# raymondclowe/EasyWakeWord

Measured on AMD Instinct MI355X. Metric: real-time 16 kHz streams sustained + MFCC frames/sec at 1/2/4/8 GPUs, higher is better.
Workload: dtype fp32

## Files before the change

### easywakeword_amd/csrc/ewk_mfcc_dft.h

```cpp
#pragma once
#include <hip/hip_runtime.h>

namespace ewk {

#define EWK_LD128(r, a, c) asm volatile("ds_read_b128 %0, %1 offset:%2" : "=v"(r[c]) : "v"(a), "i"(16 * (c)) : "memory")
#define EWK_LD128_8(r, addr)                                                                        \
    do {                                                                                           \
        const uint32_t _a = (addr);                                                                \
        EWK_LD128(r, _a, 0); EWK_LD128(r, _a, 1); EWK_LD128(r, _a, 2); EWK_LD128(r, _a, 3);         \
        EWK_LD128(r, _a, 4); EWK_LD128(r, _a, 5); EWK_LD128(r, _a, 6); EWK_LD128(r, _a, 7);         \
    } while (0)
#define EWK_WAIT_8(r)                                                                              \
    asm volatile("s_waitcnt lgkmcnt(0)" : "+v"(r[0]), "+v"(r[1]), "+v"(r[2]), "+v"(r[3]), "+v"(r[4]), \
                 "+v"(r[5]), "+v"(r[6]), "+v"(r[7]) : : "memory")

__device__ __forceinline__ float2 cmul(float2 a, float2 w) {
    return make_float2(a.x * w.x - a.y * w.y, a.x * w.y + a.y * w.x);
}

__device__ __forceinline__ void dft4(float2& a0, float2& a1, float2& a2, float2& a3) {
    const float2 t0 = make_float2(a0.x + a2.x, a0.y + a2.y);
    const float2 t1 = make_float2(a0.x - a2.x, a0.y - a2.y);
    const float2 t2 = make_float2(a1.x + a3.x, a1.y + a3.y);
    const float2 t3 = make_float2(a1.x - a3.x, a1.y - a3.y);
    a0 = make_float2(t0.x + t2.x, t0.y + t2.y);
    a2 = make_float2(t0.x - t2.x, t0.y - t2.y);
    a1 = make_float2(t1.x + t3.y, t1.y - t3.x);
    a3 = make_float2(t1.x - t3.y, t1.y + t3.x);
}

__device__ __forceinline__ void dft16_stage2(float2 (&x)[16]) {
    constexpr float C1 = 0.92387953251128674f, R2 = 0.70710678118654752f, T = 0.41421356237309505f;
    dft4(x[0], x[1], x[2], x[3]);
    {
        const float2 a0 = x[4], y1 = x[5], y2 = x[6], y3 = x[7];
        const float2 u2 = make_float2(y2.x + y2.y, y2.y - y2.x);
        const float2 t0 = make_float2(fmaf(R2, u2.x, a0.x), fmaf(R2, u2.y, a0.y));
        const float2 t1 = make_float2(fmaf(-R2, u2.x, a0.x), fmaf(-R2, u2.y, a0.y));
        const float2 u1 = make_float2(fmaf(T, y1.y, y1.x), fmaf(-T, y1.x, y1.y));
        const float2 u3 = make_float2(fmaf(T, y3.x, y3.y), fmaf(T, y3.y, -y3.x));
        const float2 v2 = make_float2(u1.x + u3.x, u1.y + u3.y), v3 = make_float2(u1.x - u3.x, u1.y - u3.y);
        x[4] = make_float2(fmaf(C1, v2.x, t0.x), fmaf(C1, v2.y, t0.y));
        x[6] = make_float2(fmaf(-C1, v2.x, t0.x), fmaf(-C1, v2.y, t0.y));
        x[5] = make_float2(fmaf(C1, v3.y, t1.x), fmaf(-C1, v3.x, t1.y));
        x[7] = make_float2(fmaf(-C1, v3.y, t1.x), fmaf(C1, v3.x, t1.y));
    }
    {
        const float2 a0 = x[8], y1 = x[9], y2 = x[10], y3 = x[11];
        const float2 t0 = make_float2(a0.x + y2.y, a0.y - y2.x);
        const float2 t1 = make_float2(a0.x - y2.y, a0.y + y2.x);
        const float2 u1 = make_float2(y1.x + y1.y, y1.y - y1.x);
        const float d3 = y3.y - y3.x, n3 = y3.x + y3.y;
        const float2 v2 = make_float2(u1.x + d3, u1.y - n3), v3 = make_float2(u1.x - d3, u1.y + n3);
        x[8] = make_float2(fmaf(R2, v2.x, t0.x), fmaf(R2, v2.y, t0.y));
        x[10] = make_float2(fmaf(-R2, v2.x, t0.x), fmaf(-R2, v2.y, t0.y));
        x[9] = make_float2(fmaf(R2, v3.y, t1.x), fmaf(-R2, v3.x, t1.y));
        x[11] = make_float2(fmaf(-R2, v3.y, t1.x), fmaf(R2, v3.x, t1.y));
    }
    {
        const float2 a0 = x[12], y1 = x[13], y2 = x[14], y3 = x[15];
        const float d2 = y2.y - y2.x, n2 = y2.x + y2.y;
        const float2 t0 = make_float2(fmaf(R2, d2, a0.x), fmaf(-R2, n2, a0.y));
        const float2 t1 = make_float2(fmaf(-R2, d2, a0.x), fmaf(R2, n2, a0.y));
        const float2 u1 = make_float2(fmaf(T, y1.x, y1.y), fmaf(T, y1.y, -y1.x));
        const float m3 = fmaf(T, y3.y, y3.x), u3y = fmaf(T, y3.x, -y3.y);
        const float2 v2 = make_float2(u1.x - m3, u1.y + u3y), v3 = make_float2(u1.x + m3, u1.y - u3y);
        x[12] = make_float2(fmaf(C1, v2.x, t0.x), fmaf(C1, v2.y, t0.y));
        x[14] = make_float2(fmaf(-C1, v2.x, t0.x), fmaf(-C1, v2.y, t0.y));
        x[13] = make_float2(fmaf(C1, v3.y, t1.x), fmaf(-C1, v3.x, t1.y));
        x[15] = make_float2(fmaf(-C1, v3.y, t1.x), fmaf(C1, v3.x, t1.y));
    }
}

__device__ __forceinline__ void dft16_perm(float2 (&x)[16]) {
#pragma unroll
    for (int n2 = 0; n2 < 4; ++n2) dft4(x[n2], x[4 + n2], x[8 + n2], x[12 + n2]);
    dft16_stage2(x);
}

__device__ __forceinline__ void dft16_perm_win(float2 (&x)[16], const float2 (&w)[16]) {
#pragma unroll
    for (int n2 = 0; n2 < 4; ++n2) {
        const float2 x0 = x[n2], x1 = x[4 + n2], x2 = x[8 + n2], x3 = x[12 + n2];
        const float2 w0 = w[n2], w1 = w[4 + n2], w2 = w[8 + n2], w3 = w[12 + n2];
        const float2 p2 = make_float2(x2.x * w2.x, x2.y * w2.y), p3 = make_float2(x3.x * w3.x, x3.y * w3.y);
        const float2 t0 = make_float2(fmaf(x0.x, w0.x, p2.x), fmaf(x0.y, w0.y, p2.y));
        const float2 t1 = make_float2(fmaf(x0.x, w0.x, -p2.x), fmaf(x0.y, w0.y, -p2.y));
        const float2 t2 = make_float2(fmaf(x1.x, w1.x, p3.x), fmaf(x1.y, w1.y, p3.y));
        const float2 t3 = make_float2(fmaf(x1.x, w1.x, -p3.x), fmaf(x1.y, w1.y, -p3.y));
        x[n2] = make_float2(t0.x + t2.x, t0.y + t2.y);
        x[8 + n2] = make_float2(t0.x - t2.x, t0.y - t2.y);
        x[4 + n2] = make_float2(t1.x + t3.y, t1.y - t3.x);
        x[12 + n2] = make_float2(t1.x - t3.y, t1.y + t3.x);
    }
    dft16_stage2(x);
}

__device__ __forceinline__ constexpr int dperm(int k) { return 4 * (k & 3) + (k >> 2); }

}
```

### easywakeword_amd/csrc/ewk_mfcc_fft.h

```cpp
#pragma once
#include <hip/hip_runtime.h>
#include <math.h>

#include "ewk_internal.h"
#include "ewk_mfcc_layout.h"
#include "ewk_mfcc_dft.h"
#include "ewk_mfcc_tile.h"

#define EWK_SETPRIO(v) __builtin_amdgcn_s_setprio(v)

namespace ewk {

__host__ __device__ constexpr int tr_off(int r, int h) {
    const int jp = r < 8 ? r : (r == 8 ? 0 : 16 - r);
    const int q = (jp >> 2) + (r >= 8 ? 2 : 0);
    return 64 * (16 * h + 4 * (jp & 3) + q) + 4 * ((jp & 3) + 8 * h);
}

template <int RING>
struct SegSrc {
    __amdgpu_buffer_rsrc_t rsrc;
    int32_t len;
    int32_t wrap_at;
    int32_t start;
    int32_t ring;
};

constexpr int sample_bytes(int ring) { return ring == 2 ? 2 : 4; }

template <int RING>
__device__ __forceinline__ SegSrc<RING> make_src(const void* p, int64_t start, int64_t ring, int32_t len) {
    SegSrc<RING> v;
    const unsigned char* b = static_cast<const unsigned char*>(p) + (RING ? 0 : start * sample_bytes(RING));
    const uint64_t bu = (uint64_t)b;
    const uint32_t lo = __builtin_amdgcn_readfirstlane((uint32_t)bu);
    const uint32_t hi = __builtin_amdgcn_readfirstlane((uint32_t)(bu >> 32));
    const void* bb = (const void*)(((uint64_t)hi << 32) | lo);
    const int32_t n = __builtin_amdgcn_readfirstlane(RING ? (int32_t)ring : len);
    v.rsrc = __builtin_amdgcn_make_buffer_rsrc((void*)bb, (short)0, n * sample_bytes(RING), 0x00020000);
    v.len = __builtin_amdgcn_readfirstlane(len);
    v.start = __builtin_amdgcn_readfirstlane((int32_t)start);
    v.ring = __builtin_amdgcn_readfirstlane((int32_t)ring);
    v.wrap_at = v.ring - v.start;
    return v;
}

template <int RING>
__device__ __forceinline__ void stage_load(const SegSrc<RING>& v, int q0, int lane, float (&r)[kStageLoads]) {
#pragma unroll
    for (int c = 0; c < kStageLoads; ++c) {
        const int q = q0 + 64 * c + lane;
        int off;
        if (RING) {
            const int phys = q >= v.wrap_at ? q - v.wrap_at : q + v.start;
            off = (unsigned)q < (unsigned)v.len ? phys * sample_bytes(RING) : -1;
        } else {
            off = q * 4;
        }
        if (RING == 2)
            r[c] = (float)(short)__builtin_amdgcn_raw_buffer_load_b16(v.rsrc, off, 0, 0);
        else
            r[c] = __builtin_bit_cast(float, __builtin_amdgcn_raw_buffer_load_b32(v.rsrc, off, 0, 0));
    }
}

#define EWK_ST13(o)                                                                                            \
    asm volatile("s_mov_b32 %[sv], m0\n\ts_mov_b32 m0, %[base]\n\ts_nop 0\n\t"                              \
                 "ds_write_addtid_b32 %[r0] offset:%[o0]\n\tds_write_addtid_b32 %[r1] offset:%[o1]\n\t"          \
                 "ds_write_addtid_b32 %[r2] offset:%[o2]\n\tds_write_addtid_b32 %[r3] offset:%[o3]\n\t"          \
                 "ds_write_addtid_b32 %[r4] offset:%[o4]\n\tds_write_addtid_b32 %[r5] offset:%[o5]\n\t"          \
                 "ds_write_addtid_b32 %[r6] offset:%[o6]\n\tds_write_addtid_b32 %[r7] offset:%[o7]\n\t"          \
                 "ds_write_addtid_b32 %[r8] offset:%[o8]\n\tds_write_addtid_b32 %[r9] offset:%[o9]\n\t"          \
                 "ds_write_addtid_b32 %[r10] offset:%[o10]\n\tds_write_addtid_b32 %[r11] offset:%[o11]\n\t"      \
                 "ds_write_addtid_b32 %[r12] offset:%[o12]\n\ts_mov_b32 m0, %[sv]"                                 \
                 : [sv] "=&s"(m0save)                                                                          \
                 : [base] "s"(m0base), [r0] "v"(r[o]), [r1] "v"(r[o + 1]), [r2] "v"(r[o + 2]), [r3] "v"(r[o + 3]), \
                   [r4] "v"(r[o + 4]), [r5] "v"(r[o + 5]), [r6] "v"(r[o + 6]), [r7] "v"(r[o + 7]),                \
                   [r8] "v"(r[o + 8]), [r9] "v"(r[o + 9]), [r10] "v"(r[o + 10]), [r11] "v"(r[o + 11]),          \
                   [r12] "v"(r[o + 12]), [o0] "i"(stg_off(o)), [o1] "i"(stg_off(o + 1)), [o2] "i"(stg_off(o + 2)), \
                   [o3] "i"(stg_off(o + 3)), [o4] "i"(stg_off(o + 4)), [o5] "i"(stg_off(o + 5)),                    \
                   [o6] "i"(stg_off(o + 6)), [o7] "i"(stg_off(o + 7)), [o8] "i"(stg_off(o + 8)),                    \
                   [o9] "i"(stg_off(o + 9)), [o10] "i"(stg_off(o + 10)), [o11] "i"(stg_off(o + 11)),                \
                   [o12] "i"(stg_off(o + 12))                                                                     \
                 : "memory")
static_assert(kStageLoads == 26, "stage_store writes two blocks of 13 rows");
__device__ __forceinline__ void stage_store(float* stage, int lane, const float (&r)[kStageLoads]) {
    const uint32_t m0base = __builtin_amdgcn_readfirstlane((uint32_t)(uintptr_t)stage);
    uint32_t m0save;
    EWK_ST13(0);
    EWK_ST13(13);
}

constexpr int kMelW[8] = {2, 2, 2, 3, 4, 6, 9, 12};
constexpr int kMelIt0[8] = {0, 2, 4, 6, 9, 13, 19, 28};
constexpr int kMelOff[8] = {0, 2, 4, 8, 12, 16, 24, 36};
constexpr int kMelRow = 48;
static_assert(kMelRow <= WP && WP % 4 == 0, "mel weight rows");

template <int G>
__device__ __forceinline__ void xpose_write(const float2 (&ag)[16], int half, uint32_t m0base) {
    constexpr int g = G;
    float w[16];
#pragma unroll
    for (int k1 = 0; k1 < 16; ++k1) w[k1] = half ? ag[dperm(k1)].y : ag[dperm(k1)].x;
    uint32_t m0save;
    asm volatile("s_mov_b32 %[sv], m0\n\ts_mov_b32 m0, %[base]\n\ts_nop 0\n\t"
                 "ds_write_addtid_b32 %[w0] offset:%[o0]\n\tds_write_addtid_b32 %[w1] offset:%[o1]\n\t"
                 "ds_write_addtid_b32 %[w2] offset:%[o2]\n\tds_write_addtid_b32 %[w3] offset:%[o3]\n\t"
                 "ds_write_addtid_b32 %[w4] offset:%[o4]\n\tds_write_addtid_b32 %[w5] offset:%[o5]\n\t"
                 "ds_write_addtid_b32 %[w6] offset:%[o6]\n\tds_write_addtid_b32 %[w7] offset:%[o7]\n\t"
                 "ds_write_addtid_b32 %[w8] offset:%[o8]\n\tds_write_addtid_b32 %[w9] offset:%[o9]\n\t"
                 "ds_write_addtid_b32 %[w10] offset:%[o10]\n\tds_write_addtid_b32 %[w11] offset:%[o11]\n\t"
                 "ds_write_addtid_b32 %[w12] offset:%[o12]\n\tds_write_addtid_b32 %[w13] offset:%[o13]\n\t"
                 "ds_write_addtid_b32 %[w14] offset:%[o14]\n\tds_write_addtid_b32 %[w15] offset:%[o15]\n\t"
                 "s_mov_b32 m0, %[sv]"
                 : [sv] "=&s"(m0save)
                 : [base] "s"(m0base), [w0] "v"(w[0]), [w1] "v"(w[1]), [w2] "v"(w[2]), [w3] "v"(w[3]),
                   [w4] "v"(w[4]), [w5] "v"(w[5]), [w6] "v"(w[6]), [w7] "v"(w[7]), [w8] "v"(w[8]),
                   [w9] "v"(w[9]), [w10] "v"(w[10]), [w11] "v"(w[11]), [w12] "v"(w[12]),
                   [w13] "v"(w[13]), [w14] "v"(w[14]), [w15] "v"(w[15]),
                   [o0] "i"(4 * tr_off(0, g)), [o1] "i"(4 * tr_off(1, g)), [o2] "i"(4 * tr_off(2, g)),
                   [o3] "i"(4 * tr_off(3, g)), [o4] "i"(4 * tr_off(4, g)), [o5] "i"(4 * tr_off(5, g)),
                   [o6] "i"(4 * tr_off(6, g)), [o7] "i"(4 * tr_off(7, g)), [o8] "i"(4 * tr_off(8, g)),
                   [o9] "i"(4 * tr_off(9, g)), [o10] "i"(4 * tr_off(10, g)), [o11] "i"(4 * tr_off(11, g)),
                   [o12] "i"(4 * tr_off(12, g)), [o13] "i"(4 * tr_off(13, g)), [o14] "i"(4 * tr_off(14, g)),
                   [o15] "i"(4 * tr_off(15, g))
                 : "memory");
}

template <int RING>
__device__ __forceinline__ void frame_pass(const SegSrc<RING>& v, int t0, int T, int row0, int next_t0,
                                           const unsigned char* smem, float* scr, float* tile,
                                           int lane, const int (&lo)[8], float& vmax, float& vmin, float& nanp,
                                           float clampv EWK_PASS_PARAM) {
    EWK_TS(fp0);
    EWK_SETPRIO(1);
    const int f = lane >> 4, j = lane & 15;
    const int jp = j & 7;
    const int rowA = jp, rowB = jp ? 16 - jp : 8;
    float* scf = scr + scr_frame_off(4 * (j >> 3) + f);
    bool valid[kNF];
    float* sc[kNF];
#pragma unroll
    for (int g = 0; g < kNF; ++g) {
        valid[g] = t0 + 2 * f + g < T;
        sc[g] = scr + scr_frame_off(4 * g + f);
    }

    float2 a[kNF][16];
    floatx4 t4[8];
    {
        float2 x[kNF][16];
        {
            const uint32_t sa = (uint32_t)(uintptr_t)(scr + 352 * f + 2 * j);
#define EWK_LD64(g, n) asm volatile("ds_read_b64 %0, %1 offset:%2" : "=v"(x[g][n]) : "v"(sa), "i"(win_off(g, n)) : "memory")
            EWK_LD64(0, 0); EWK_LD64(0, 1); EWK_LD64(0, 2); EWK_LD64(0, 3); EWK_LD64(0, 4); EWK_LD64(0, 5);
            EWK_LD64(0, 6); EWK_LD64(0, 7); EWK_LD64(0, 8); EWK_LD64(0, 9); EWK_LD64(0, 10); EWK_LD64(0, 11);
            EWK_LD64(0, 12); EWK_LD64(0, 13); EWK_LD64(0, 14); EWK_LD64(0, 15);
            EWK_LD64(1, 11); EWK_LD64(1, 12); EWK_LD64(1, 13); EWK_LD64(1, 14); EWK_LD64(1, 15);
#undef EWK_LD64
        }
        floatx4 w4[8];
        EWK_LD128_8(w4, (uint32_t)(uintptr_t)(reinterpret_cast<const float4*>(smem + L_WIN2) + j * (TP / 2)));
        EWK_WAIT_8(w4);
        asm volatile("s_waitcnt lgkmcnt(0)"
                     : "+v"(x[0][0]), "+v"(x[0][1]), "+v"(x[0][2]), "+v"(x[0][3]), "+v"(x[0][4]), "+v"(x[0][5]),
                       "+v"(x[0][6]), "+v"(x[0][7]), "+v"(x[0][8]), "+v"(x[0][9]), "+v"(x[0][10]), "+v"(x[0][11]),
                       "+v"(x[0][12]), "+v"(x[0][13]), "+v"(x[0][14]), "+v"(x[0][15])
                     :
                     : "memory");
        asm volatile("s_waitcnt lgkmcnt(0)"
                     : "+v"(x[1][11]), "+v"(x[1][12]), "+v"(x[1][13]), "+v"(x[1][14]), "+v"(x[1][15])
                     :
                     : "memory");
#pragma unroll
        for (int n = 0; n <= 10; ++n) x[1][n] = x[0][n + 5];
        float2 wv[16];
#pragma unroll
        for (int c = 0; c < 8; ++c) {
            wv[2 * c] = make_float2(w4[c].x, w4[c].y);
            wv[2 * c + 1] = make_float2(w4[c].z, w4[c].w);
        }
        EWK_SETPRIO(0);
        EWK_LD128_8(t4, (uint32_t)(uintptr_t)(reinterpret_cast<const float4*>(smem + L_TW1) + j * (TP / 2)));
#pragma unroll
        for (int g = 0; g < kNF; ++g) {
#pragma unroll
            for (int n = 0; n < 16; ++n) a[g][n] = x[g][n];
            dft16_perm_win(a[g], wv);
        }
    }
    lds_order();
    EWK_TS(fp1);
    float pf[kStageLoads];
    {
        EWK_WAIT_8(t4);
#pragma unroll
        for (int c = 0; c < 8; ++c) {
            const floatx4 w = t4[c];
#pragma unroll
            for (int g = 0; g < kNF; ++g) {
                a[g][dperm(2 * c + 1)] = cmul(a[g][dperm(2 * c + 1)], make_float2(w.x, w.y));
                if (c < 7) a[g][dperm(2 * c + 2)] = cmul(a[g][dperm(2 * c + 2)], make_float2(w.z, w.w));
            }
        }
    }
    EWK_TS(fp2);
    EWK_SETPRIO(1);
    float2 b[kNF][16];
    {
        const uint32_t m0base = __builtin_amdgcn_readfirstlane((uint32_t)(uintptr_t)scr);
        const int offA = tr_off(rowA, j >> 3) + 16 * f, offB = tr_off(rowB, j >> 3) + 16 * f;
#pragma unroll
        for (int half = 0; half < 2; ++half) {
#pragma unroll
            for (int g = 0; g < kNF; ++g) {
                if (g == 0) xpose_write<0>(a[0], half, m0base);
                else xpose_write<1>(a[1], half, m0base);
            }
            lds_order();
#pragma unroll
            for (int s2 = 0; s2 < 2; ++s2) {
                const float4* rd = reinterpret_cast<const float4*>(scr + (s2 ? offB : offA));
#pragma unroll
                for (int c = 0; c < 4; ++c) {
                    const float4 q = rd[c];
                    if (half) {
                        b[s2][4 * c].y = q.x; b[s2][4 * c + 1].y = q.y; b[s2][4 * c + 2].y = q.z; b[s2][4 * c + 3].y = q.w;
                    } else {
                        b[s2][4 * c].x = q.x; b[s2][4 * c + 1].x = q.y; b[s2][4 * c + 2].x = q.z; b[s2][4 * c + 3].x = q.w;
                    }
                }
            }
            lds_order();
        }
    }
    EWK_TS(fp3);
    EWK_SETPRIO(0);
#pragma unroll
    for (int g = 0; g < kNF; ++g) dft16_perm(b[g]);
    EWK_TS(fp4);
    {
        const bool z0 = jp == 0;
        float2 tw[18];
        {
            const float4* t4 = reinterpret_cast<const float4*>(smem + L_TW2) + jp * (TP / 2);
#pragma unroll
            for (int c = 0; c < 9; ++c) {
                const float4 q = t4[c];
                tw[2 * c] = make_float2(q.x, q.y);
                tw[2 * c + 1] = make_float2(q.z, q.w);
            }
        }
        float* pA0 = scf + rowA;
        float* pA1 = z0 ? scf - 136 : pA0;
        float* pA2 = z0 ? scf - 136 : pA0 - 16;
        float* pB0 = scf - rowA;
        float* pB1 = z0 ? scf + 136 : pB0;
        float* pB2 = z0 ? scf + 136 : pB0 + 16;
#pragma unroll
        for (int it0 = 0; it0 < 17; it0 += 2) {
            float py[2], px[2];
#pragma unroll
            for (int u = 0; u < 2; ++u) {
                const int it = it0 + u;
                if (it >= 17) break;
                const float2 w = tw[it];
                const float2 ug = b[0][dperm(it < 16 ? it : 15)];
                const float2 vg = b[1][dperm(it < 16 ? 15 - it : 0)];
                float2 uu, vv;
                if (it <= 8) {
                    uu = ug;
                    const float2 vz = b[0][dperm((16 - it) & 15)];
                    vv = z0 ? vz : vg;
                } else {
                    const float2 uz = b[1][dperm(it - 9)], vz = b[1][dperm(24 - it)];
                    uu = z0 ? uz : ug;
                    vv = z0 ? vz : vg;
                }
                const float ar = uu.x + vv.x, ai = uu.y - vv.y;
                const float br = uu.x - vv.x, bi = uu.y + vv.y;
                const float er = fmaf(w.y, br, -bi), ei = fmaf(w.y, bi, br);
                const float yr = fmaf(-w.x, er, ar), yi = fmaf(-w.x, ei, ai);
                const float xr = fmaf(w.x, er, ar), xi = fmaf(w.x, ei, ai);
                py[u] = yr * yr + yi * yi;
                px[u] = xr * xr + xi * xi;
            }
#pragma unroll
            for (int u = 0; u < 2; ++u) {
                const int it = it0 + u;
                if (it >= 17) break;
                float* pa = it <= 8 ? pA0 : (it < 16 ? pA1 : pA2);
                pa[16 * it] = py[u];
            }
#pragma unroll
            for (int u = 0; u < 2; ++u) {
                const int it = it0 + u;
                if (it >= 17) break;
                float* pb = it <= 8 ? pB0 : (it < 16 ? pB1 : pB2);
                pb[256 - 16 * it] = px[u];
            }
        }
        scf[257 + jp] = 0.0f;
        if (jp < 7) scf[265 + jp] = 0.0f;
    }
    lds_order();
    EWK_TS(fp5);
    EWK_SETPRIO(1);
    if (next_t0 >= 0) stage_load(v, next_t0 * HOP - NFFT / 2, lane, pf);
    float db[kNF][8];
    {
        const float* wrow = reinterpret_cast<const float*>(smem + L_WPAD) + j * WP;
#pragma unroll
        for (int hh = 0; hh < 2; ++hh) {
            const int i0 = hh ? 6 : 0, i1 = hh ? 8 : 6;
            float wv[MEL_ITERS], pv[kNF][MEL_ITERS];
#pragma unroll
            for (int i = i0; i < i1; ++i) {
                if (kMelW[i] <= 2) {
                    const float2 w = *reinterpret_cast<const float2*>(wrow + kMelOff[i]);
                    wv[kMelIt0[i]] = w.x; wv[kMelIt0[i] + 1] = w.y;
                } else {
#pragma unroll
                    for (int c = 0; c < (kMelW[i] + 3) / 4; ++c) {
                        const float4 w = *reinterpret_cast<const float4*>(wrow + kMelOff[i] + 4 * c);
                        const float ww[4] = {w.x, w.y, w.z, w.w};
#pragma unroll
                        for (int e = 0; e < 4; ++e)
                            if (4 * c + e < kMelW[i]) wv[kMelIt0[i] + 4 * c + e] = ww[e];
                    }
                }
#pragma unroll
                for (int g = 0; g < kNF; ++g) {
                    const float* sp = sc[g] + lo[i];
#pragma unroll
                    for (int q = 0; q < kMelW[i]; ++q) pv[g][kMelIt0[i] + q] = sp[q];
                }
            }
#pragma unroll
            for (int i = i0; i < i1; ++i)
#pragma unroll
                for (int g = 0; g < kNF; ++g) {
                    float acc = 0.0f;
#pragma unroll
                    for (int q = 0; q < kMelW[i]; ++q) acc = fmaf(wv[kMelIt0[i] + q], pv[g][kMelIt0[i] + q], acc);
                    db[g][i] = 3.0102999566398120f * __log2f(fmaxf(1e-10f, acc));
                    if (i == 0) nanp = fmaf(acc, 0.0f, nanp);
                }
        }
    }
    EWK_SETPRIO(0);
    lds_order();
    EWK_TS(fp6);
#pragma unroll
    for (int g = 0; g < kNF; ++g) {
        const int r = row0 + 2 * f + g;
        float fmx = db[g][0], fmn = db[g][0], x[8];
#pragma unroll
        for (int i = 0; i < 8; ++i) {
            fmx = fmaxf(fmx, db[g][i]);
            fmn = fminf(fmn, db[g][i]);
            x[i] = fmaxf(db[g][i], clampv);
        }
        vmax = fmaxf(vmax, valid[g] ? fmx : -INFINITY);
        vmin = fminf(vmin, valid[g] ? fmn : INFINITY);
        uint4 hi, lo;
        split8(x, hi, lo);
        unsigned char* tb = reinterpret_cast<unsigned char*>(tile) + tile_chunk(r, j);
        *reinterpret_cast<uint4*>(tb) = hi;
        *reinterpret_cast<uint4*>(tb + 256) = lo;
    }
    lds_order();
    if (next_t0 >= 0) stage_store(scr, lane, pf);
    lds_order();
#ifdef EWK_TIMING
    EWK_TS(fp7);
    if (pdbg) {
        pdbg[12] += fp1 - fp0; pdbg[13] += fp2 - fp1; pdbg[14] += fp3 - fp2; pdbg[15] += fp4 - fp3;
        pdbg[16] += fp5 - fp4; pdbg[17] += fp6 - fp5; pdbg[18] += fp7 - fp6; pdbg[19] += 1;
    }
#endif
}

}
```

Before: 2.854 billion.

## Replace full LDS waits with graded lgkmcnt waits in window, twiddle and mel stages

The window stage now issues the window-weight reads first and loads frame samples in butterfly-group order. It waits on partial lgkmcnt counts so each radix-4 group can start as soon as its inputs arrive, instead of waiting for every read. The twiddle multiply waits per twiddle vector, and the mel filterbank is unrolled into hand-written ds_read sequences with staged partial waits, so LDS latency overlaps with FMA/log work. The cost is brittle hand-counted waitcnt values, guarded by static_asserts on the band widths and offsets. A miscount or any compiler-inserted LDS op could cause races or extra stalls.

```diff
diff --git a/easywakeword_amd/csrc/ewk_mfcc_dft.h b/easywakeword_amd/csrc/ewk_mfcc_dft.h
--- a/easywakeword_amd/csrc/ewk_mfcc_dft.h
+++ b/easywakeword_amd/csrc/ewk_mfcc_dft.h
@@ -10,9 +10,13 @@
         EWK_LD128(r, _a, 0); EWK_LD128(r, _a, 1); EWK_LD128(r, _a, 2); EWK_LD128(r, _a, 3);         \
         EWK_LD128(r, _a, 4); EWK_LD128(r, _a, 5); EWK_LD128(r, _a, 6); EWK_LD128(r, _a, 7);         \
     } while (0)
-#define EWK_WAIT_8(r)                                                                              \
-    asm volatile("s_waitcnt lgkmcnt(0)" : "+v"(r[0]), "+v"(r[1]), "+v"(r[2]), "+v"(r[3]), "+v"(r[4]), \
-                 "+v"(r[5]), "+v"(r[6]), "+v"(r[7]) : : "memory")
+
+#define EWK_V(r) "+v"(r)
+#define EWK_WAIT_N(n, ...)                                                                          \
+    do {                                                                                           \
+        static_assert((n) >= 0 && (n) <= 15, "lgkmcnt counts to 15");                             \
+        asm volatile("s_waitcnt lgkmcnt(%[cnt])" : __VA_ARGS__ : [cnt] "i"(n) : "memory");         \
+    } while (0)
 
 __device__ __forceinline__ float2 cmul(float2 a, float2 w) {
     return make_float2(a.x * w.x - a.y * w.y, a.x * w.y + a.y * w.x);
@@ -78,21 +82,23 @@
     dft16_stage2(x);
 }
 
+__device__ __forceinline__ void dft16_win_group(float2 (&x)[16], const float2 (&w)[16], int n2) {
+    const float2 x0 = x[n2], x1 = x[4 + n2], x2 = x[8 + n2], x3 = x[12 + n2];
+    const float2 w0 = w[n2], w1 = w[4 + n2], w2 = w[8 + n2], w3 = w[12 + n2];
+    const float2 p2 = make_float2(x2.x * w2.x, x2.y * w2.y), p3 = make_float2(x3.x * w3.x, x3.y * w3.y);
+    const float2 t0 = make_float2(fmaf(x0.x, w0.x, p2.x), fmaf(x0.y, w0.y, p2.y));
+    const float2 t1 = make_float2(fmaf(x0.x, w0.x, -p2.x), fmaf(x0.y, w0.y, -p2.y));
+    const float2 t2 = make_float2(fmaf(x1.x, w1.x, p3.x), fmaf(x1.y, w1.y, p3.y));
+    const float2 t3 = make_float2(fmaf(x1.x, w1.x, -p3.x), fmaf(x1.y, w1.y, -p3.y));
+    x[n2] = make_float2(t0.x + t2.x, t0.y + t2.y);
+    x[8 + n2] = make_float2(t0.x - t2.x, t0.y - t2.y);
+    x[4 + n2] = make_float2(t1.x + t3.y, t1.y - t3.x);
+    x[12 + n2] = make_float2(t1.x - t3.y, t1.y + t3.x);
+}
+
 __device__ __forceinline__ void dft16_perm_win(float2 (&x)[16], const float2 (&w)[16]) {
 #pragma unroll
-    for (int n2 = 0; n2 < 4; ++n2) {
-        const float2 x0 = x[n2], x1 = x[4 + n2], x2 = x[8 + n2], x3 = x[12 + n2];
-        const float2 w0 = w[n2], w1 = w[4 + n2], w2 = w[8 + n2], w3 = w[12 + n2];
-        const float2 p2 = make_float2(x2.x * w2.x, x2.y * w2.y), p3 = make_float2(x3.x * w3.x, x3.y * w3.y);
-        const float2 t0 = make_float2(fmaf(x0.x, w0.x, p2.x), fmaf(x0.y, w0.y, p2.y));
-        const float2 t1 = make_float2(fmaf(x0.x, w0.x, -p2.x), fmaf(x0.y, w0.y, -p2.y));
-        const float2 t2 = make_float2(fmaf(x1.x, w1.x, p3.x), fmaf(x1.y, w1.y, p3.y));
-        const float2 t3 = make_float2(fmaf(x1.x, w1.x, -p3.x), fmaf(x1.y, w1.y, -p3.y));
-        x[n2] = make_float2(t0.x + t2.x, t0.y + t2.y);
-        x[8 + n2] = make_float2(t0.x - t2.x, t0.y - t2.y);
-        x[4 + n2] = make_float2(t1.x + t3.y, t1.y - t3.x);
-        x[12 + n2] = make_float2(t1.x - t3.y, t1.y + t3.x);
-    }
+    for (int n2 = 0; n2 < 4; ++n2) dft16_win_group(x, w, n2);
     dft16_stage2(x);
 }
 
diff --git a/easywakeword_amd/csrc/ewk_mfcc_fft.h b/easywakeword_amd/csrc/ewk_mfcc_fft.h
--- a/easywakeword_amd/csrc/ewk_mfcc_fft.h
+++ b/easywakeword_amd/csrc/ewk_mfcc_fft.h
@@ -150,53 +150,70 @@
     float2 a[kNF][16];
     floatx4 t4[8];
     {
+        floatx4 w4[8];
+        EWK_LD128_8(w4, (uint32_t)(uintptr_t)(reinterpret_cast<const float4*>(smem + L_WIN2) + j * (TP / 2)));
         float2 x[kNF][16];
         {
             const uint32_t sa = (uint32_t)(uintptr_t)(scr + 352 * f + 2 * j);
 #define EWK_LD64(g, n) asm volatile("ds_read_b64 %0, %1 offset:%2" : "=v"(x[g][n]) : "v"(sa), "i"(win_off(g, n)) : "memory")
-            EWK_LD64(0, 0); EWK_LD64(0, 1); EWK_LD64(0, 2); EWK_LD64(0, 3); EWK_LD64(0, 4); EWK_LD64(0, 5);
-            EWK_LD64(0, 6); EWK_LD64(0, 7); EWK_LD64(0, 8); EWK_LD64(0, 9); EWK_LD64(0, 10); EWK_LD64(0, 11);
-            EWK_LD64(0, 12); EWK_LD64(0, 13); EWK_LD64(0, 14); EWK_LD64(0, 15);
+            EWK_LD64(0, 0); EWK_LD64(0, 4); EWK_LD64(0, 8); EWK_LD64(0, 12);
+            EWK_LD64(0, 1); EWK_LD64(0, 5); EWK_LD64(0, 9); EWK_LD64(0, 13);
+            EWK_LD64(0, 2); EWK_LD64(0, 6); EWK_LD64(0, 10); EWK_LD64(0, 14);
+            EWK_LD64(0, 3); EWK_LD64(0, 7); EWK_LD64(0, 11); EWK_LD64(0, 15);
             EWK_LD64(1, 11); EWK_LD64(1, 12); EWK_LD64(1, 13); EWK_LD64(1, 14); EWK_LD64(1, 15);
 #undef EWK_LD64
         }
-        floatx4 w4[8];
-        EWK_LD128_8(w4, (uint32_t)(uintptr_t)(reinterpret_cast<const float4*>(smem + L_WIN2) + j * (TP / 2)));
-        EWK_WAIT_8(w4);
-        asm volatile("s_waitcnt lgkmcnt(0)"
-                     : "+v"(x[0][0]), "+v"(x[0][1]), "+v"(x[0][2]), "+v"(x[0][3]), "+v"(x[0][4]), "+v"(x[0][5]),
-                       "+v"(x[0][6]), "+v"(x[0][7]), "+v"(x[0][8]), "+v"(x[0][9]), "+v"(x[0][10]), "+v"(x[0][11]),
-                       "+v"(x[0][12]), "+v"(x[0][13]), "+v"(x[0][14]), "+v"(x[0][15])
-                     :
-                     : "memory");
-        asm volatile("s_waitcnt lgkmcnt(0)"
-                     : "+v"(x[1][11]), "+v"(x[1][12]), "+v"(x[1][13]), "+v"(x[1][14]), "+v"(x[1][15])
-                     :
-                     : "memory");
-#pragma unroll
-        for (int n = 0; n <= 10; ++n) x[1][n] = x[0][n + 5];
+#define EWK_WAIT_GROUP(n2, ...)                                                                        \
+        EWK_WAIT_N((4 * (3 - (n2)) + 5 > 15 ? 15 : 4 * (3 - (n2)) + 5), EWK_V(x[0][n2]), EWK_V(x[0][4 + (n2)]), \
+                   EWK_V(x[0][8 + (n2)]), EWK_V(x[0][12 + (n2)]) __VA_ARGS__)
+        EWK_WAIT_GROUP(0, , EWK_V(w4[0]), EWK_V(w4[1]), EWK_V(w4[2]), EWK_V(w4[3]), EWK_V(w4[4]), EWK_V(w4[5]),
+                       EWK_V(w4[6]), EWK_V(w4[7]));
+        EWK_SETPRIO(0);
         float2 wv[16];
 #pragma unroll
         for (int c = 0; c < 8; ++c) {
             wv[2 * c] = make_float2(w4[c].x, w4[c].y);
             wv[2 * c + 1] = make_float2(w4[c].z, w4[c].w);
         }
-        EWK_SETPRIO(0);
+#define EWK_GROUP(n2)                                                                                  \
+        a[0][n2] = x[0][n2]; a[0][4 + (n2)] = x[0][4 + (n2)]; a[0][8 + (n2)] = x[0][8 + (n2)];         \
+        a[0][12 + (n2)] = x[0][12 + (n2)];                                                             \
+        dft16_win_group(a[0], wv, n2)
+        EWK_GROUP(0);
+        EWK_WAIT_GROUP(1);
+        EWK_GROUP(1);
+        EWK_WAIT_GROUP(2);
+        EWK_GROUP(2);
+        EWK_WAIT_GROUP(3);
+        EWK_GROUP(3);
+#undef EWK_GROUP
+#undef EWK_WAIT_GROUP
         EWK_LD128_8(t4, (uint32_t)(uintptr_t)(reinterpret_cast<const float4*>(smem + L_TW1) + j * (TP / 2)));
-#pragma unroll
-        for (int g = 0; g < kNF; ++g) {
-#pragma unroll
-            for (int n = 0; n < 16; ++n) a[g][n] = x[g][n];
-            dft16_perm_win(a[g], wv);
-        }
-    }
+        dft16_stage2(a[0]);
+        EWK_WAIT_N(8, EWK_V(x[1][11]), EWK_V(x[1][12]), EWK_V(x[1][13]), EWK_V(x[1][14]), EWK_V(x[1][15]));
+#pragma unroll
+        for (int n = 0; n <= 10; ++n) x[1][n] = x[0][n + 5];
+#pragma unroll
+        for (int n = 0; n < 16; ++n) a[1][n] = x[1][n];
+        dft16_perm_win(a[1], wv);
+    }
+    static_assert(kNF == 2, "the window stage's waits count the reads of two frames per lane");
     lds_order();
     EWK_TS(fp1);
     float pf[kStageLoads];
     {
-        EWK_WAIT_8(t4);
 #pragma unroll
         for (int c = 0; c < 8; ++c) {
+            switch (c) {
+                case 0: EWK_WAIT_N(7, EWK_V(t4[0])); break;
+                case 1: EWK_WAIT_N(6, EWK_V(t4[1])); break;
+                case 2: EWK_WAIT_N(5, EWK_V(t4[2])); break;
+                case 3: EWK_WAIT_N(4, EWK_V(t4[3])); break;
+                case 4: EWK_WAIT_N(3, EWK_V(t4[4])); break;
+                case 5: EWK_WAIT_N(2, EWK_V(t4[5])); break;
+                case 6: EWK_WAIT_N(1, EWK_V(t4[6])); break;
+                default: EWK_WAIT_N(0, EWK_V(t4[7])); break;
+            }
             const floatx4 w = t4[c];
 #pragma unroll
             for (int g = 0; g < kNF; ++g) {
@@ -310,44 +327,142 @@
     if (next_t0 >= 0) stage_load(v, next_t0 * HOP - NFFT / 2, lane, pf);
     float db[kNF][8];
     {
-        const float* wrow = reinterpret_cast<const float*>(smem + L_WPAD) + j * WP;
-#pragma unroll
-        for (int hh = 0; hh < 2; ++hh) {
-            const int i0 = hh ? 6 : 0, i1 = hh ? 8 : 6;
-            float wv[MEL_ITERS], pv[kNF][MEL_ITERS];
-#pragma unroll
-            for (int i = i0; i < i1; ++i) {
-                if (kMelW[i] <= 2) {
-                    const float2 w = *reinterpret_cast<const float2*>(wrow + kMelOff[i]);
-                    wv[kMelIt0[i]] = w.x; wv[kMelIt0[i] + 1] = w.y;
-                } else {
-#pragma unroll
-                    for (int c = 0; c < (kMelW[i] + 3) / 4; ++c) {
-                        const float4 w = *reinterpret_cast<const float4*>(wrow + kMelOff[i] + 4 * c);
-                        const float ww[4] = {w.x, w.y, w.z, w.w};
-#pragma unroll
-                        for (int e = 0; e < 4; ++e)
-                            if (4 * c + e < kMelW[i]) wv[kMelIt0[i] + 4 * c + e] = ww[e];
-                    }
-                }
-#pragma unroll
-                for (int g = 0; g < kNF; ++g) {
-                    const float* sp = sc[g] + lo[i];
-#pragma unroll
-                    for (int q = 0; q < kMelW[i]; ++q) pv[g][kMelIt0[i] + q] = sp[q];
-                }
-            }
-#pragma unroll
-            for (int i = i0; i < i1; ++i)
-#pragma unroll
-                for (int g = 0; g < kNF; ++g) {
-                    float acc = 0.0f;
-#pragma unroll
-                    for (int q = 0; q < kMelW[i]; ++q) acc = fmaf(wv[kMelIt0[i] + q], pv[g][kMelIt0[i] + q], acc);
-                    db[g][i] = 3.0102999566398120f * __log2f(fmaxf(1e-10f, acc));
-                    if (i == 0) nanp = fmaf(acc, 0.0f, nanp);
-                }
-        }
+        static_assert(kNF == 2 && kMelW[0] == 2 && kMelW[1] == 2 && kMelW[2] == 2 && kMelW[3] == 3 && kMelW[4] == 4 &&
+                          kMelW[5] == 6 && kMelW[6] == 9 && kMelW[7] == 12 && kMelOff[1] == 2 && kMelOff[2] == 4 &&
+                          kMelOff[3] == 8 && kMelOff[4] == 12 && kMelOff[5] == 16 && kMelOff[6] == 24 && kMelOff[7] == 36,
+                      "the mel stage's reads are written out for these group widths and row offsets");
+        const uint32_t wa = (uint32_t)(uintptr_t)(reinterpret_cast<const float*>(smem + L_WPAD) + j * WP);
+        const uint32_t scb[kNF] = {(uint32_t)(uintptr_t)sc[0], (uint32_t)(uintptr_t)sc[1]};
+        uint32_t pa[kNF][8];
+#define EWK_MKPA(i)                                                                                   \
+        asm volatile("v_lshl_add_u32 %0, %1, 2, %2" : "=v"(pa[0][i]) : "v"(lo[i]), "v"(scb[0]));      \
+        asm volatile("v_lshl_add_u32 %0, %1, 2, %2" : "=v"(pa[1][i]) : "v"(lo[i]), "v"(scb[1]))
+#define EWK_PA(g, i) pa[g][i]
+#define EWK_RD2(d, a, q) asm volatile("ds_read2_b32 %0, %1 offset0:%2 offset1:%3" : "=v"(d) : "v"(a), "i"(q), "i"((q) + 1) : "memory")
+#define EWK_RD1(d, a, q) asm volatile("ds_read_b32 %0, %1 offset:%2" : "=v"(d) : "v"(a), "i"(4 * (q)) : "memory")
+#define EWK_RD64(d, a, q) asm volatile("ds_read_b64 %0, %1 offset:%2" : "=v"(d) : "v"(a), "i"(4 * (q)) : "memory")
+#define EWK_RD128(d, a, q) asm volatile("ds_read_b128 %0, %1 offset:%2" : "=v"(d) : "v"(a), "i"(4 * (q)) : "memory")
+#define EWK_MEL_GROUP(i, W)                                                                          \
+        _Pragma("unroll") for (int g = 0; g < kNF; ++g) {                                            \
+            float acc = 0.0f;                                                                        \
+            _Pragma("unroll") for (int q = 0; q < W; ++q) acc = fmaf(w[q], p[g][q], acc);            \
+            db[g][i] = 3.0102999566398120f * __log2f(fmaxf(1e-10f, acc));                            \
+            if (i == 0) nanp = fmaf(acc, 0.0f, nanp);                                                \
+        }
+#define EWK_MEL_BAND(i, g, W, w)                                                                      \
+        {                                                                                            \
+            float acc = 0.0f;                                                                        \
+            _Pragma("unroll") for (int q = 0; q < W; ++q) acc = fmaf(w[q], p[q], acc);               \
+            db[g][i] = 3.0102999566398120f * __log2f(fmaxf(1e-10f, acc));                            \
+        }
+        floatx4 wA, wC, wD, wE, wG[3], wH[3];
+        float2 wB, wF;
+        float2 p0[kNF], p1[kNF], p2[kNF], p3[kNF], p4[kNF][2], p5[kNF][3], p6[kNF][4], p7[kNF][6];
+        float p3s[kNF], p6s[kNF];
+        EWK_RD128(wA, wa, 0); EWK_RD64(wB, wa, 4);
+        EWK_MKPA(0);
+        EWK_RD2(p0[0], EWK_PA(0, 0), 0); EWK_RD2(p0[1], EWK_PA(1, 0), 0);
+        EWK_MKPA(1);
+        EWK_RD2(p1[0], EWK_PA(0, 1), 0); EWK_RD2(p1[1], EWK_PA(1, 1), 0);
+        EWK_MKPA(2);
+        EWK_RD2(p2[0], EWK_PA(0, 2), 0); EWK_RD2(p2[1], EWK_PA(1, 2), 0);
+        EWK_RD128(wC, wa, 8);
+        EWK_MKPA(3);
+        EWK_RD2(p3[0], EWK_PA(0, 3), 0); EWK_RD1(p3s[0], EWK_PA(0, 3), 2);
+        EWK_RD2(p3[1], EWK_PA(1, 3), 0); EWK_RD1(p3s[1], EWK_PA(1, 3), 2);
+        EWK_RD128(wD, wa, 12);
+        EWK_MKPA(4);
+        EWK_RD2(p4[0][0], EWK_PA(0, 4), 0); EWK_RD2(p4[0][1], EWK_PA(0, 4), 2);
+        EWK_RD2(p4[1][0], EWK_PA(1, 4), 0); EWK_RD2(p4[1][1], EWK_PA(1, 4), 2);
+        EWK_WAIT_N(10, EWK_V(wA), EWK_V(wB), EWK_V(p0[0]), EWK_V(p0[1]), EWK_V(p1[0]), EWK_V(p1[1]), EWK_V(p2[0]),
+                   EWK_V(p2[1]));
+        {
+            const float w[2] = {wA.x, wA.y}, p[kNF][2] = {{p0[0].x, p0[0].y}, {p0[1].x, p0[1].y}};
+            EWK_MEL_GROUP(0, 2)
+        }
+        {
+            const float w[2] = {wA.z, wA.w}, p[kNF][2] = {{p1[0].x, p1[0].y}, {p1[1].x, p1[1].y}};
+            EWK_MEL_GROUP(1, 2)
+        }
+        {
+            const float w[2] = {wB.x, wB.y}, p[kNF][2] = {{p2[0].x, p2[0].y}, {p2[1].x, p2[1].y}};
+            EWK_MEL_GROUP(2, 2)
+        }
+        EWK_RD128(wE, wa, 16); EWK_RD64(wF, wa, 20);
+        EWK_MKPA(5);
+        EWK_RD2(p5[0][0], EWK_PA(0, 5), 0); EWK_RD2(p5[0][1], EWK_PA(0, 5), 2); EWK_RD2(p5[0][2], EWK_PA(0, 5), 4);
+        EWK_RD2(p5[1][0], EWK_PA(1, 5), 0); EWK_RD2(p5[1][1], EWK_PA(1, 5), 2); EWK_RD2(p5[1][2], EWK_PA(1, 5), 4);
+        EWK_WAIT_N(13, EWK_V(wC), EWK_V(p3[0]), EWK_V(p3s[0]), EWK_V(p3[1]), EWK_V(p3s[1]));
+        {
+            const float w[3] = {wC.x, wC.y, wC.z};
+            const float p[kNF][3] = {{p3[0].x, p3[0].y, p3s[0]}, {p3[1].x, p3[1].y, p3s[1]}};
+            EWK_MEL_GROUP(3, 3)
+        }
+        EWK_WAIT_N(8, EWK_V(wD), EWK_V(p4[0][0]), EWK_V(p4[0][1]), EWK_V(p4[1][0]), EWK_V(p4[1][1]));
+        {
+            const float w[4] = {wD.x, wD.y, wD.z, wD.w};
+            const float p[kNF][4] = {{p4[0][0].x, p4[0][0].y, p4[0][1].x, p4[0][1].y},
+                                     {p4[1][0].x, p4[1][0].y, p4[1][1].x, p4[1][1].y}};
+            EWK_MEL_GROUP(4, 4)
+        }
+        EWK_RD128(wG[0], wa, 24); EWK_RD128(wG[1], wa, 28); EWK_RD128(wG[2], wa, 32);
+        EWK_MKPA(6);
+        EWK_RD2(p6[0][0], EWK_PA(0, 6), 0); EWK_RD2(p6[0][1], EWK_PA(0, 6), 2); EWK_RD2(p6[0][2], EWK_PA(0, 6), 4);
+        EWK_RD2(p6[0][3], EWK_PA(0, 6), 6); EWK_RD1(p6s[0], EWK_PA(0, 6), 8);
+        EWK_WAIT_N(8, EWK_V(wE), EWK_V(wF), EWK_V(p5[0][0]), EWK_V(p5[0][1]), EWK_V(p5[0][2]), EWK_V(p5[1][0]),
+                   EWK_V(p5[1][1]), EWK_V(p5[1][2]));
+        {
+            const float w[6] = {wE.x, wE.y, wE.z, wE.w, wF.x, wF.y};
+            const float p[kNF][6] = {{p5[0][0].x, p5[0][0].y, p5[0][1].x, p5[0][1].y, p5[0][2].x, p5[0][2].y},
+                                     {p5[1][0].x, p5[1][0].y, p5[1][1].x, p5[1][1].y, p5[1][2].x, p5[1][2].y}};
+            EWK_MEL_GROUP(5, 6)
+        }
+        EWK_RD2(p6[1][0], EWK_PA(1, 6), 0); EWK_RD2(p6[1][1], EWK_PA(1, 6), 2); EWK_RD2(p6[1][2], EWK_PA(1, 6), 4);
+        EWK_RD2(p6[1][3], EWK_PA(1, 6), 6); EWK_RD1(p6s[1], EWK_PA(1, 6), 8);
+        EWK_WAIT_N(5, EWK_V(wG[0]), EWK_V(wG[1]), EWK_V(wG[2]), EWK_V(p6[0][0]), EWK_V(p6[0][1]), EWK_V(p6[0][2]),
+                   EWK_V(p6[0][3]), EWK_V(p6s[0]));
+        const float w6[9] = {wG[0].x, wG[0].y, wG[0].z, wG[0].w, wG[1].x, wG[1].y, wG[1].z, wG[1].w, wG[2].x};
+        {
+            const float p[9] = {p6[0][0].x, p6[0][0].y, p6[0][1].x, p6[0][1].y, p6[0][2].x, p6[0][2].y, p6[0][3].x,
+                                p6[0][3].y, p6s[0]};
+            EWK_MEL_BAND(6, 0, 9, w6)
+        }
+        EWK_RD128(wH[0], wa, 36); EWK_RD128(wH[1], wa, 40); EWK_RD128(wH[2], wa, 44);
+        EWK_MKPA(7);
+        EWK_RD2(p7[0][0], EWK_PA(0, 7), 0); EWK_RD2(p7[0][1], EWK_PA(0, 7), 2); EWK_RD2(p7[0][2], EWK_PA(0, 7), 4);
+        EWK_RD2(p7[0][3], EWK_PA(0, 7), 6); EWK_RD2(p7[0][4], EWK_PA(0, 7), 8); EWK_RD2(p7[0][5], EWK_PA(0, 7), 10);
+        EWK_WAIT_N(9, EWK_V(p6[1][0]), EWK_V(p6[1][1]), EWK_V(p6[1][2]), EWK_V(p6[1][3]), EWK_V(p6s[1]));
+        {
+            const float p[9] = {p6[1][0].x, p6[1][0].y, p6[1][1].x, p6[1][1].y, p6[1][2].x, p6[1][2].y, p6[1][3].x,
+                                p6[1][3].y, p6s[1]};
+            EWK_MEL_BAND(6, 1, 9, w6)
+        }
+        EWK_RD2(p7[1][0], EWK_PA(1, 7), 0); EWK_RD2(p7[1][1], EWK_PA(1, 7), 2); EWK_RD2(p7[1][2], EWK_PA(1, 7), 4);
+        EWK_RD2(p7[1][3], EWK_PA(1, 7), 6); EWK_RD2(p7[1][4], EWK_PA(1, 7), 8); EWK_RD2(p7[1][5], EWK_PA(1, 7), 10);
+        EWK_WAIT_N(6, EWK_V(wH[0]), EWK_V(wH[1]), EWK_V(wH[2]), EWK_V(p7[0][0]), EWK_V(p7[0][1]), EWK_V(p7[0][2]),
+                   EWK_V(p7[0][3]), EWK_V(p7[0][4]), EWK_V(p7[0][5]));
+        const float w7[12] = {wH[0].x, wH[0].y, wH[0].z, wH[0].w, wH[1].x, wH[1].y, wH[1].z, wH[1].w,
+                              wH[2].x, wH[2].y, wH[2].z, wH[2].w};
+        {
+            const float p[12] = {p7[0][0].x, p7[0][0].y, p7[0][1].x, p7[0][1].y, p7[0][2].x, p7[0][2].y, p7[0][3].x,
+                                 p7[0][3].y, p7[0][4].x, p7[0][4].y, p7[0][5].x, p7[0][5].y};
+            EWK_MEL_BAND(7, 0, 12, w7)
+        }
+        EWK_WAIT_N(0, EWK_V(p7[1][0]), EWK_V(p7[1][1]), EWK_V(p7[1][2]), EWK_V(p7[1][3]), EWK_V(p7[1][4]),
+                   EWK_V(p7[1][5]));
+        {
+            const float p[12] = {p7[1][0].x, p7[1][0].y, p7[1][1].x, p7[1][1].y, p7[1][2].x, p7[1][2].y, p7[1][3].x,
+                                 p7[1][3].y, p7[1][4].x, p7[1][4].y, p7[1][5].x, p7[1][5].y};
+            EWK_MEL_BAND(7, 1, 12, w7)
+        }
+#undef EWK_MEL_BAND
+#undef EWK_MEL_GROUP
+#undef EWK_RD128
+#undef EWK_RD64
+#undef EWK_RD1
+#undef EWK_RD2
+#undef EWK_PA
+#undef EWK_MKPA
     }
     EWK_SETPRIO(0);
     lds_order();
```

New measurement: 2.868 billion (median of 6 runs). About the same (+0.5%).
